# cudagu/aero-gnn

Hardware: AMD Instinct MI355X
Metric: million edge-updates/sec, 1M-node/6M-edge mesh, 1->8 MI355X (higher is better)
Workload: dtype bf16; 1 GPU; BSMS-MGN 4-scale U-Net train step (fwd+MSE+bwd+allreduce+Adam), 1000000 nodes / 5996000 edges per GPU; model=BiStridedMeshGraphNet(H=128, n_hid=2, processor_size=15, stride=2, concat_trick), mode=train, global_batch=1, parallelism=dp1

## Files before the change

### aero-gnn_amd/aerognn/_lib.py

```python
from __future__ import annotations

import ctypes as C
import os

_HERE = os.path.dirname(os.path.abspath(__file__))
LIB_PATH = os.environ.get("AEROGNN_LIB") or os.path.join(_HERE, "libaerognn.so")

MAX_LIN = 8
MAX_SEG = 3
F32, BF16, F16, F64 = 0, 1, 2, 3
SEG_PLAIN, SEG_GATHER, SEG_SUM, SEG_MEAN = 0, 1, 2, 3
OPT_RESIDENT = 0

vp = C.c_void_p
i32 = C.c_int


class Seg(C.Structure):
    _fields_ = [("kind", i32), ("k", i32), ("ld", i32), ("_pad", i32),
                ("ptr", vp), ("index", vp), ("store", vp)]


ACT = {"relu": 0, "gelu": 1, "silu": 2, "tanh": 3}

# ... 17 lines not shown
                ("hpre", vp), ("stats", vp), ("ln_g", vp),
                ("g", vp), ("g2", vp), ("gidx", vp),
                ("gpre", vp * MAX_LIN),
                ("din_nseg", i32), ("din_k", i32 * MAX_SEG),
                ("din", vp * MAX_SEG), ("din_resid", i32 * MAX_SEG),
                ("ln_partial", vp), ("tiled", i32), ("gpre_tiled", i32),
                ("mask", vp * MAX_LIN), ("act_fn", i32), ("_pad3", i32), ("pre", vp * MAX_LIN)]


MAX_WGRAD = 8


class WgradDesc(C.Structure):
    _fields_ = [("g", vp), ("x", vp), ("ldg", i32), ("ldx", i32), ("m", i32), ("k", i32), ("rows", i32),
                ("ldw", i32), ("dw_partial", vp), ("db_partial", vp), ("dw", vp), ("db", vp),
                ("g_tiled", i32), ("x_tiled", i32), ("nsplit", i32), ("_pad", i32), ("xidx", vp)]


class WgradBatch(C.Structure):
    _fields_ = [("n", i32), ("_pad", i32), ("d", WgradDesc * MAX_WGRAD)]


class WecArgs(C.Structure):
    _fields_ = [("n", i32), ("e", i32), ("dtype", i32), ("out_dim", i32), ("hid", i32), ("pos_dim", i32),
                ("pos_ld", i32), ("mean", i32),
                ("rowptr", vp), ("src", vp), ("dst", vp), ("perm", vp), ("rowptr_src", vp), ("perm_src", vp),
                ("pos", vp), ("pab", vp), ("tx", vp), ("w1c", vp), ("w2", vp),
                ("w_in", vp), ("w_out", vp), ("out", vp), ("dout", vp), ("gw", vp), ("s_csc", vp), ("dh", vp),
                ("dpa", vp), ("dpb", vp), ("dtx", vp), ("dw_in", vp), ("partial", vp)]


# ... 199 lines not shown
```

### aero-gnn_amd/aerognn/core.py

```python
from __future__ import annotations

import ctypes as C

import torch

from . import _lib as L
from ._lib import check, ptr


def stream():
    return C.c_void_p(torch.cuda.current_stream().cuda_stream)


PROF = None
_TIMED_DEPTH = 0


class _Timed:
    __slots__ = ("tag", "cost", "s", "on")

    def __init__(self, tag, cost):
        self.tag, self.cost = tag, cost
        self.on = False

# ... 477 lines not shown


def scatter_rows(idx32, src, out):
    check(L.lib().agn_scatter_rows(idx32.numel(), src.shape[1], dt_code(src.dtype), ptr(idx32), ptr(src),
                                   src.stride(0), ptr(out), out.stride(0), stream()), "scatter_rows")
    return out


def colsum_rows(p, nw, n, out):
    sr = min(512, max(1, nw))
    scratch = torch.empty(sr * n, dtype=torch.float32, device=p.device)
    check(L.lib().agn_colsum(ptr(p), nw, n, ptr(scratch), sr, ptr(out), stream()), "colsum")
    return out


class WGrad:

    def __init__(self, tag="wgrad"):
        self.items = []
        self.tag = tag

    def add(self, G, X, dw, db=None, xidx=None):
        assert G.dtype == X.dtype and logical_rows(G) == (logical_rows(X) if xidx is None else xidx.numel())
        assert dw.dtype == torch.float32 and dw.stride(1) == 1
        assert xidx is None or (xidx.dtype == torch.int32 and not is_tiled(X))
        self.items.append((G, X, dw, db, xidx))

    def run(self):
        lib = L.lib()
        plain = [it for it in self.items if it[4] is None]
        gath = [it for it in self.items if it[4] is not None]
        chunks = [grp[i:i + L.MAX_WGRAD] for grp in (plain, gath) for i in range(0, len(grp), L.MAX_WGRAD)]
        for chunk in chunks:
            dev = chunk[0][0].device
            live = []
            for G, X, dw, db, xi in chunk:
                if logical_rows(G) == 0:
                    dw.zero_()
                    if db is not None:
                        db.zero_()
                else:
                    live.append((G, X, dw, db, xi))
            if not live:
                continue
            b = L.WgradBatch()
            b.n = len(live)
            for j, (G, X, dw, db, xi) in enumerate(live):
                b.d[j] = L.WgradDesc(ptr(G), ptr(X), G.stride(0), X.stride(0), G.shape[1], X.shape[1], logical_rows(G),
                                     dw.stride(0), None, None, ptr(dw), ptr(db), int(is_tiled(G)), int(is_tiled(X)), 0, 0,
                                     ptr(xi))
            check(lib.agn_wgrad_plan(C.byref(b)), "wgrad_plan")
            sizes = [int(lib.agn_wgrad_partial_floats(G.shape[1], X.shape[1], b.d[j].nsplit))
                     for j, (G, X, _, _, _) in enumerate(live)]
            bsz = [b.d[j].nsplit * ((G.shape[1] + 127) // 128) * 128 if db is not None else 0
                   for j, (G, _, _, db, _) in enumerate(live)]
            scratch = torch.empty(sum(sizes) + sum(bsz), dtype=torch.float32, device=dev)
            o = 0
            for j, (G, X, dw, db, _) in enumerate(live):
                b.d[j].dw_partial = ptr(scratch[o:o + sizes[j]])
                o += sizes[j]
                if db is not None:
                    b.d[j].db_partial = ptr(scratch[o:o + bsz[j]])
                    o += bsz[j]
            s_el = live[0][0].element_size()
            io = sum(logical_rows(G) * (G.shape[1] + X.shape[1]) * s_el + 4 * G.shape[1] * (X.shape[1] + 1)
                     for G, X, _, _, _ in live)
            fl = sum(2.0 * logical_rows(G) * G.shape[1] * X.shape[1] for G, X, _, _, _ in live)
            with timed(self.tag, (0.0, fl, io)):
                check(lib.agn_wgrad(C.byref(b), dt_code(live[0][0].dtype), 0, stream()), "wgrad")
        self.items = []


def alg8d_edge(E, N, H, s, bwd=False):
    return (2 if bwd else 1) * (E * (2 * s * H + 8) + N * 2 * s * H)


def alg8d_node(N, H, s, bwd=False, proj=False):
    return (2 if bwd else 1) * N * 3 * s * H * (2 if (bwd and proj) else 1)


def with_alg(alg, impl):
    return (alg, impl[1], impl[0])


# ... 57 lines not shown
```

### aero-gnn_amd/aerognn/functions.py

```python
from __future__ import annotations

import ctypes as C

import torch

from . import _lib as L
from ._lib import check, ptr
from . import core as _core
from .core import (Pack, WGrad, alg8d_edge, alg8d_node, with_alg, edge_bwd_fused, fused_edge_train_ok, bwd_nblocks,
                   edge32_ok, edge_saves_ok, edge_forward,
                   cost_edge_bwd_fused,
                   proj_kernel_ok, proj_forward, proj_backward, tiled_empty, relu_mask_empty, colsum_rows, cost_edge_bwd, cost_edge_bwd_cat, cost_edge_fwd,
                   cost_edge_fwd_cat, cost_node_bwd, cost_node_fwd, cost_proj, cost_wec_bwd, cost_wec_fwd, dt_code,
                   timed, gather_rows, mlp_backward, mlp_forward, require_device,
                   scatter_rows, segment_max, segment_max_backward, segment_sum, segment_sum2, stream)


def _c(t):
    return t if t.is_contiguous() else t.contiguous()


def _ln_grads(partial, nblk, M, dtype):
    out = torch.empty(2 * M, dtype=torch.float32, device=partial.device)
    colsum_rows(partial, nblk, 2 * M, out)
# ... 73 lines not shown
        stats = torch.empty(rows, 2, dtype=torch.float32, device=dev)
    return acts, hpre, stats


def _alloc_gpre(spec, rows, dtype, dev, rowmajor=()):
    out = []
    for l in range(spec.nlin):
        w = spec.hidden if l < spec.nlin - 1 else spec.out_dim
        if w == spec.hidden == 128 and l not in rowmajor:
            out.append(tiled_empty(rows, w, dtype, dev))
        else:
            out.append(torch.empty(rows, w, dtype=dtype, device=dev))
    return out


def _chain_param_grads(spec, gpre, inputs0, acts, lnp_partial, nblk, wg=None, tag="wgrad_enc"):
    own = wg is None
    wg = wg or WGrad(tag)
    grads = []
    dev = gpre[0].device
    for l, (w, b) in enumerate(spec.linears):
        G = gpre[l]
        M, K = w.shape
        dw = torch.empty(M, K, dtype=torch.float32, device=dev)
        db = torch.empty(M, dtype=torch.float32, device=dev) if b is not None else None
        if l == 0 and isinstance(inputs0, (list, tuple)):
            k0 = 0
            for j, X in enumerate(inputs0):
                X, xi = X if isinstance(X, tuple) else (X, None)
                wg.add(G, X, dw[:, k0:k0 + X.shape[1]], db if j == 0 else None, xidx=xi)
                k0 += X.shape[1]
        else:
            wg.add(G, inputs0 if l == 0 else acts[l - 1], dw, db)
        grads.append((dw, w.dtype))
        if b is not None:
            grads.append((db, b.dtype))
    if own:
        wg.run()
    out = [g if g.dtype == dt else g.to(dt) for g, dt in grads]
    if spec.ln is not None:
        g, bb = _ln_grads(lnp_partial, nblk, spec.out_dim, spec.ln[0].dtype)
# ... 332 lines not shown
                dxs = torch.empty(E, H, dtype=dt, device=dev)
                dxd = torch.empty(E, H, dtype=dt, device=dev)
                din = [(H, dxs, False), (H, dxd, False), (H, de, True)] if spec.gmp_order else \
                    [(H, de, True), (H, dxs, False), (H, dxd, False)]
            nb_e = mlp_backward(rows=E, dtype=dt, hidden=H, nlin=es.nlin, act_fn=es.act, out_dim=H, in_dim=es.in_dim,
                                wtpk=es.wtpk(), acts=ea, g=ge, g2=dagg, gidx=lv.dst, gpre=gpre_e,
                                ln_g=es.lnp()[0] if es.ln else None, hpre=ehp, stats=est, din=din, ln_partial=part_e,
                                tag="edge_bwd",
                                cost=with_alg(alg8d_edge(E, N, H, sz, bwd=True),
                                              (cost_edge_bwd if spec.trick else cost_edge_bwd_cat)(E, N, H, sz,
                                                                                                   es.nlin)))
            g0 = gpre_e[0]
        grads_edge = []
        if spec.trick:
            dPs = segment_sum(N, H, lv.rowptr_src, lv.perm_src, g0, torch.empty(N, H, dtype=dt, device=dev))
            dPd = segment_sum(N, H, lv.rowptr, None, g0, torch.empty(N, H, dtype=dt, device=dev))
            if proj_kernel_ok(dx, H):
                s_el = dx.element_size()
                proj_backward(N, dPs, dPd, spec.pack["projT"], dx, tag="proj_bwd",
                              cost=with_alg(alg8d_node(N, H, s_el, bwd=True), (4 * N * H * s_el, 4.0 * N * H * H)))
            else:
                mlp_forward(rows=N, dtype=dt, hidden=H, nlin=1, out_dim=H,
                            segs=[(L.SEG_PLAIN, H, H, dPs, None, None), (L.SEG_PLAIN, H, H, dPd, None, None)],
                            wpk=[spec.pack["projT"]], bias=[None], resid=dx, out=dx)
            eb = spec.eb
            wg = WGrad("wgrad_node")
            if fused:
                dwe = torch.empty(H, H, dtype=torch.float32, device=dev)
                we = WGrad("wgrad_edge")
                we.add(g0, e, dwe)
                we.run()
                eg = [dwe]
                for l in range(3):
                    eg += [dW13[l], db13[l]]
                eg = eg[:1] + [t if t.dtype == p.dtype else t.to(p.dtype) for t, p in zip(eg[1:], es.params()[1:7])]
                eg += list(_ln_grads(part_e, nb_e, H, es.ln[0].dtype))
            else:
                eg = _chain_param_grads(es, gpre_e, e, ea, part_e, nb_e, tag="wgrad_edge")
            dws = torch.empty(H, x.shape[1], dtype=torch.float32, device=dev)
            dwd = torch.empty(H, x.shape[1], dtype=torch.float32, device=dev)
            dbd = torch.empty(H, dtype=torch.float32, device=dev)
            wg.add(dPs, x, dws)
            wg.add(dPd, x, dwd, dbd)
            grads_node = _chain_param_grads(ns, gpre_n, [x, agg], na, part_n, nb_n, wg)
            wg.run()
            if fused and eg[0].dtype != es.linears[0][0].dtype:
                eg[0] = eg[0].to(es.linears[0][0].dtype)
            grads_edge = [eg[0], dws.to(eb.src_lin.dtype), dwd.to(eb.dst_lin.dtype), dbd.to(eb.bias.dtype)] + eg[1:]
            return (dx, de, None, None, None, *grads_edge, *grads_node)
        else:
            segment_sum2(N, H, dx, (lv.rowptr_src, lv.perm_src, dxs), (lv.rowptr, None, dxd), dx)
            xs, xd = (x, lv.src), (x, lv.dst)
            grads_edge = _chain_param_grads(es, gpre_e, [xs, xd, e] if spec.gmp_order else [e, xs, xd],
# ... 141 lines not shown
        nb = bwd_nblocks(E)
        part = torch.empty(nb, 2 * H, dtype=torch.float32, device=dev) if es.ln else None
        de = torch.empty_like(e)
        if spec.trick:
            din = [(H, de, False)]
        else:
            dxs = torch.empty(E, H, dtype=dt, device=dev)
            dxd = torch.empty(E, H, dtype=dt, device=dev)
            din = [(H, de, False), (H, dxs, False), (H, dxd, False)]
        nb = mlp_backward(rows=E, dtype=dt, hidden=H, nlin=es.nlin, act_fn=es.act, out_dim=H, in_dim=es.in_dim, wtpk=es.wtpk(),
                     acts=ea, g=g, gpre=gpre, ln_g=es.lnp()[0] if es.ln else None, hpre=ehp, stats=est,
                     din=din, ln_partial=part)
        if spec.trick:
            g0 = gpre[0]
            dPs = segment_sum(N, H, lv.rowptr_src, lv.perm_src, g0, torch.empty(N, H, dtype=dt, device=dev))
            dPd = segment_sum(N, H, lv.rowptr, None, g0, torch.empty(N, H, dtype=dt, device=dev))
            dx = torch.zeros_like(x)
            mlp_forward(rows=N, dtype=dt, hidden=H, nlin=1, out_dim=H,
                        segs=[(L.SEG_PLAIN, H, H, dPs, None, None), (L.SEG_PLAIN, H, H, dPd, None, None)],
                        wpk=[spec.pack["projT"]], bias=[None], out=dx)
            eg = _chain_param_grads(es, gpre, e, ea, part, nb, tag="wgrad_edge")
            eb = spec.eb
            wg = WGrad("wgrad_node")
            dws = torch.empty(H, x.shape[1], dtype=torch.float32, device=dev)
            dwd = torch.empty(H, x.shape[1], dtype=torch.float32, device=dev)
            dbd = torch.empty(H, dtype=torch.float32, device=dev)
            wg.add(dPs, x, dws)
            wg.add(dPd, x, dwd, dbd)
            wg.run()
            grads = [eg[0], dws.to(eb.src_lin.dtype), dwd.to(eb.dst_lin.dtype), dbd.to(eb.bias.dtype)] + eg[1:]
        else:
            dx = segment_sum2(N, H, None, (lv.rowptr_src, lv.perm_src, dxs), (lv.rowptr, None, dxd),
                              torch.empty(N, H, dtype=dt, device=dev))
            grads = _chain_param_grads(es, gpre, [e, (x, lv.src), (x, lv.dst)], ea, part, nb, tag="wgrad_edge")
        return (dx, de, None, None, None, *grads)

# ... 321 lines not shown
```

### aero-gnn_amd/csrc/dw.hip

```cpp
#include "common.hpp"
#include "aerognn.h"

#include <type_traits>

using namespace agn;

namespace {

#ifndef AGN_DW_ROWS
#define AGN_DW_ROWS 64
#endif
constexpr int DW_ROWS = AGN_DW_ROWS;
constexpr int DW_BLK = 128;
constexpr int DW_THREADS = 256;

typedef short s16x4 __attribute__((ext_vector_type(4)));
typedef __attribute__((address_space(3))) s16x4 lds_s16x4;

template <typename T> struct DwTile;
template <> struct DwTile<bf16> { static constexpr int LD = 136; };
template <> struct DwTile<f16> { static constexpr int LD = 136; };
template <> struct DwTile<float> { static constexpr int LD = 132; };

template <typename T>
// ... 57 lines not shown
#pragma unroll
            for (int e = 0; e < 4; ++e)
              if (4 + e < nv) e4[e] = p[4 + e];
            const u32x2 hi = *reinterpret_cast<const u32x2*>(e4);
            v[j] = __builtin_bit_cast(uint4, u32x4{lo[0], lo[1], hi[0], hi[1]});
          } else {
            T e8[PER16];
#pragma unroll
            for (int e = 0; e < PER16; ++e) e8[e] = e < nv ? p[e] : from_f<T>(0.f);
            v[j] = *reinterpret_cast<const uint4*>(e8);
          }
        }
      }
    }
  }
  AGN_DEV void store(T* lds, int tiled) const {
    constexpr int LD = DwTile<T>::LD;
    if (tiled) {
#pragma unroll
      for (int j = 0; j < NCH; ++j) {
        int row, i, hh;
        tiled_pos(threadIdx.x + j * DW_THREADS, row, i, hh);
        if constexpr (sizeof(T) == 2) {
          const u32x4 x = __builtin_bit_cast(u32x4, v[j]);
          typedef uint32_t u32x2 __attribute__((ext_vector_type(2)));
          *reinterpret_cast<u32x2*>(lds + row * LD + 16 * i + 4 * hh) = u32x2{x[0], x[1]};
          *reinterpret_cast<u32x2*>(lds + row * LD + 16 * i + 8 + 4 * hh) = u32x2{x[2], x[3]};
        } else {
          *reinterpret_cast<uint4*>(lds + row * LD + 8 * i + 4 * hh) = v[j];
        }
// ... 12 lines not shown
AGN_DEV bf16x8 tr_frag(const bf16* lds, int kb, int col_base, int lane) {
  constexpr int LD = DwTile<bf16>::LD;
  const int q = (lane & 15) >> 2, p = lane & 3;
  const bf16* a0 = lds + (kb + q) * LD + col_base + 4 * p;
  const bf16* a1 = a0 + 4 * LD;
  s16x4 lo = __builtin_amdgcn_ds_read_tr16_b64_v4i16((lds_s16x4*)(a0));
  s16x4 hi = __builtin_amdgcn_ds_read_tr16_b64_v4i16((lds_s16x4*)(a1));
  bf16x8 r;
  const bf16x4 l4 = *reinterpret_cast<const bf16x4*>(&lo);
  const bf16x4 h4 = *reinterpret_cast<const bf16x4*>(&hi);
  r[0] = l4[0]; r[1] = l4[1]; r[2] = l4[2]; r[3] = l4[3];
  r[4] = h4[0]; r[5] = h4[1]; r[6] = h4[2]; r[7] = h4[3];
  return r;
}

template <typename T, bool XG>
__global__ __launch_bounds__(DW_THREADS) void wgrad_kernel(const agn_wgrad_batch b, int nsplit) {
  constexpr int LD = DwTile<T>::LD;
  __shared__ __attribute__((aligned(16))) T sg[DW_ROWS * LD];
  __shared__ __attribute__((aligned(16))) T sx[DW_ROWS * LD];
  const agn_wgrad_desc& d = b.d[blockIdx.z];
  const int nKb = (d.k + DW_BLK - 1) / DW_BLK;
  const int nMb = (d.m + DW_BLK - 1) / DW_BLK;
  if ((int)blockIdx.y >= nMb * nKb) return;
  const int mb = blockIdx.y / nKb, kb = blockIdx.y % nKb;
  const int m0 = mb * DW_BLK, k0 = kb * DW_BLK;
  const int split = blockIdx.x;
  const int per = ((d.rows + nsplit - 1) / nsplit + DW_ROWS - 1) / DW_ROWS * DW_ROWS;
  const int rbeg = split * per, rend = min(d.rows, rbeg + per);
  const int lane = threadIdx.x & 63, w = threadIdx.x >> 6;
  const int wm = (w >> 1) * 64, wk = (w & 1) * 64;
  const T* G = reinterpret_cast<const T*>(d.g);
  const T* X = reinterpret_cast<const T*>(d.x);
  f32x16 acc[2][2];
#pragma unroll
  for (int i = 0; i < 2; ++i)
#pragma unroll
    for (int j = 0; j < 2; ++j) acc[i][j] = f32x16{};
  float bsum = 0.f;
  __shared__ float bhalf[DW_BLK];
  StageRegs<T> rg, rx;
  if (rbeg < rend) {
    rg.load(G, d.ldg, rend, d.m, rbeg, m0, d.g_tiled);
    rx.load(X, d.ldx, rend, d.k, rbeg, k0, d.x_tiled, XG ? d.xidx : nullptr);
  }
  for (int r0 = rbeg; r0 < rend; r0 += DW_ROWS) {
    __syncthreads();
    rg.store(sg, d.g_tiled);
    rx.store(sx, d.x_tiled);
    __syncthreads();
    if (r0 + DW_ROWS < rend) {
      rg.load(G, d.ldg, rend, d.m, r0 + DW_ROWS, m0, d.g_tiled);
      rx.load(X, d.ldx, rend, d.k, r0 + DW_ROWS, k0, d.x_tiled, XG ? d.xidx : nullptr);
    }
    if (d.db_partial && kb == 0) {
      const int col = threadIdx.x & (DW_BLK - 1), q = threadIdx.x >> 7;
#pragma unroll
      for (int gq = 0; gq < DW_ROWS / 32; ++gq)
#pragma unroll 8
        for (int r = 0; r < 16; ++r) bsum += to_f(sg[(32 * gq + 16 * q + r) * LD + col]);
    }
    if constexpr (sizeof(T) == 2) {
#pragma unroll
      for (int ks = 0; ks < DW_ROWS; ks += 16) {
        const int kbase = ks + 8 * (lane >> 5);
        bf16x8 a[2], bb[2];
#pragma unroll
        for (int i = 0; i < 2; ++i) a[i] = tr_frag(reinterpret_cast<const bf16*>(sg), kbase, wm + 32 * i + 16 * ((lane >> 4) & 1), lane);
#pragma unroll
        for (int j = 0; j < 2; ++j) bb[j] = tr_frag(reinterpret_cast<const bf16*>(sx), kbase, wk + 32 * j + 16 * ((lane >> 4) & 1), lane);
#pragma unroll
        for (int i = 0; i < 2; ++i)
#pragma unroll
          for (int j = 0; j < 2; ++j) {
            if constexpr (std::is_same<T, f16>::value)
              acc[i][j] = __builtin_amdgcn_mfma_f32_32x32x16_f16(__builtin_bit_cast(f16x8, a[i]),
                                                                 __builtin_bit_cast(f16x8, bb[j]), acc[i][j], 0, 0, 0);
            else
              acc[i][j] = __builtin_amdgcn_mfma_f32_32x32x16_bf16(a[i], bb[j], acc[i][j], 0, 0, 0);
          }
      }
    } else {
      const float* fg = reinterpret_cast<const float*>(sg);
      const float* fx = reinterpret_cast<const float*>(sx);
#pragma unroll 4
      for (int ks = 0; ks < DW_ROWS; ks += 2) {
        const int r = ks + (lane >> 5), cidx = lane & 31;
        float a[2], bb[2];
#pragma unroll
        for (int i = 0; i < 2; ++i) a[i] = fg[r * LD + wm + 32 * i + cidx];
#pragma unroll
        for (int j = 0; j < 2; ++j) bb[j] = fx[r * LD + wk + 32 * j + cidx];
#pragma unroll
        for (int i = 0; i < 2; ++i)
#pragma unroll
          for (int j = 0; j < 2; ++j) acc[i][j] = __builtin_amdgcn_mfma_f32_32x32x2f32(a[i], bb[j], acc[i][j], 0, 0, 0);
      }
    }
  }
  const int kpad = nKb * DW_BLK;
  float* P = d.dw_partial + (size_t)split * (nMb * DW_BLK) * kpad;
#pragma unroll
  for (int i = 0; i < 2; ++i)
#pragma unroll
    for (int j = 0; j < 2; ++j)
#pragma unroll
      for (int r = 0; r < 16; ++r) {
        const int m = m0 + wm + 32 * i + (r & 3) + 8 * (r >> 2) + 4 * (lane >> 5);
        const int k = k0 + wk + 32 * j + (lane & 31);
        P[(size_t)m * kpad + k] = acc[i][j][r];
      }
  if (d.db_partial && kb == 0) {
    __syncthreads();
    if (threadIdx.x >= DW_BLK) bhalf[threadIdx.x - DW_BLK] = bsum;
    __syncthreads();
    if (threadIdx.x < DW_BLK) d.db_partial[(size_t)split * (nMb * DW_BLK) + m0 + threadIdx.x] = bsum + bhalf[threadIdx.x];
  }
}

constexpr int RED_G = 8;
constexpr int RED_Q = 16;
__global__ __launch_bounds__(RED_Q * RED_G) void wgrad_reduce_kernel(const agn_wgrad_batch b) {
  __shared__ f32x4 part[RED_G][RED_Q];
  __shared__ float bpart[RED_G][RED_Q];
  const agn_wgrad_desc& d = b.d[blockIdx.y];
  const int nsplit = d.nsplit;
  const int nKb = (d.k + DW_BLK - 1) / DW_BLK, nMb = (d.m + DW_BLK - 1) / DW_BLK;
  const int kpad = nKb * DW_BLK, mpad = nMb * DW_BLK;
  const size_t slab = (size_t)mpad * kpad;
  const int kq = kpad / 4;
  const int t = threadIdx.x % RED_Q, g = threadIdx.x / RED_Q;
  const int qidx = blockIdx.x * RED_Q + t;
  const bool in_slab = qidx < mpad * kq;
  f32x4 s = {0.f, 0.f, 0.f, 0.f};
  if (in_slab) {
    const float* p = d.dw_partial + (size_t)qidx * 4;
    int sp = g;
    for (; sp + 3 * RED_G < nsplit; sp += 4 * RED_G) {
      f32x4 v[4];
#pragma unroll
      for (int j = 0; j < 4; ++j) v[j] = *reinterpret_cast<const f32x4*>(p + (size_t)(sp + j * RED_G) * slab);
// ... 83 lines not shown
  hipError_t e = hipGetLastError();
  return e == hipSuccess ? 0 : (int)e;
}

}

extern "C" {

namespace {
int wgrad_resident() {
  static int resident = 0;
  if (resident == 0) {
    int dev = 0, ncu = 256, per = 3;
    hipDeviceProp_t p;
    if (hipGetDevice(&dev) == hipSuccess && hipGetDeviceProperties(&p, dev) == hipSuccess) ncu = p.multiProcessorCount;
    if (hipOccupancyMaxActiveBlocksPerMultiprocessor(&per, wgrad_kernel<bf16, false>, DW_THREADS, 0) != hipSuccess || per < 1)
      per = 3;
    resident = ncu * per;
  }
  return resident;
}
int out_blocks(const agn_wgrad_desc& d) { return ((d.m + DW_BLK - 1) / DW_BLK) * ((d.k + DW_BLK - 1) / DW_BLK); }
}

int agn_wgrad_nsplit(int rows, int ndesc_blocks) {
  int ns = wgrad_resident() / (ndesc_blocks > 0 ? ndesc_blocks : 1);
  const int maxs = (rows + 2 * DW_ROWS - 1) / (2 * DW_ROWS);
  if (ns > maxs) ns = maxs;
  return ns < 1 ? 1 : ns;
}

// ... 6 lines not shown
  if (!b || b->n < 1 || b->n > AGN_MAX_WGRAD) return AGN_E_ARG;
  int nblk = 0, rows = 0;
  for (int i = 0; i < b->n; ++i) {
    nblk += out_blocks(b->d[i]);
    rows = b->d[i].rows > rows ? b->d[i].rows : rows;
  }
  const int ns = agn_wgrad_nsplit(rows, nblk);
  for (int i = 0; i < b->n; ++i) b->d[i].nsplit = ns;
  return 0;
}

int agn_wgrad(const agn_wgrad_batch* b, int dtype, int nsplit, void* stream) {
  if (!b || b->n < 1 || b->n > AGN_MAX_WGRAD) return AGN_E_ARG;
  agn_wgrad_batch bb = *b;
  int total = 0, maxq = 1;
  for (int i = 0; i < bb.n; ++i) {
    agn_wgrad_desc& d = bb.d[i];
    if (d.m < 1 || d.k < 1 || d.rows < 0) return AGN_E_ARG;
    if ((d.g_tiled && d.m != DW_BLK) || (d.x_tiled && d.k != DW_BLK)) return AGN_E_SHAPE;
    if (d.xidx && d.x_tiled) return AGN_E_ARG;
    if (nsplit > 0) d.nsplit = nsplit;
    if (d.nsplit < 1) return AGN_E_ARG;
    total += out_blocks(d) * d.nsplit;
    const int kpad = ((d.k + DW_BLK - 1) / DW_BLK) * DW_BLK, mpad = ((d.m + DW_BLK - 1) / DW_BLK) * DW_BLK;
    maxq = mpad * kpad / 4 > maxq ? mpad * kpad / 4 : maxq;
  }
  hipStream_t st = (hipStream_t)stream;
  const int ns = bb.d[0].nsplit;
  int maxblk = 1;
  for (int i = 0; i < bb.n; ++i) {
    if (bb.d[i].nsplit != ns) return AGN_E_ARG;
    maxblk = out_blocks(bb.d[i]) > maxblk ? out_blocks(bb.d[i]) : maxblk;
  }
  (void)total;
  dim3 grid(ns, maxblk, bb.n);
  bool xg = false;
  for (int i = 0; i < bb.n; ++i) xg = xg || bb.d[i].xidx != nullptr;
#define AGN_WG(T)                                                                             \
  do {                                                                                        \
    if (xg) hipLaunchKernelGGL((wgrad_kernel<T, true>), grid, dim3(DW_THREADS), 0, st, bb, ns); \
    else hipLaunchKernelGGL((wgrad_kernel<T, false>), grid, dim3(DW_THREADS), 0, st, bb, ns);   \
  } while (0)
  if (dtype == AGN_BF16) AGN_WG(bf16);
  else if (dtype == AGN_F16) AGN_WG(f16);
  else if (dtype == AGN_F32) AGN_WG(float);
  else return AGN_E_DTYPE;
#undef AGN_WG
  hipLaunchKernelGGL(wgrad_reduce_kernel, dim3((maxq + RED_Q - 1) / RED_Q, bb.n), dim3(RED_Q * RED_G), 0, st, bb);
  return launch_status();
}

int agn_wgrad_reduce(const agn_wgrad_batch* b, int nsplit, void* stream) {
  if (!b || b->n < 1 || b->n > AGN_MAX_WGRAD || nsplit < 1) return AGN_E_ARG;
  agn_wgrad_batch bb = *b;
  int maxq = 1;
  for (int i = 0; i < bb.n; ++i) {
    bb.d[i].nsplit = nsplit;
    const int kpad = ((bb.d[i].k + DW_BLK - 1) / DW_BLK) * DW_BLK;
    const int mpad = ((bb.d[i].m + DW_BLK - 1) / DW_BLK) * DW_BLK;
    maxq = mpad * kpad / 4 > maxq ? mpad * kpad / 4 : maxq;
  }
  hipLaunchKernelGGL(wgrad_reduce_kernel, dim3((maxq + RED_Q - 1) / RED_Q, bb.n), dim3(RED_Q * RED_G), 0, (hipStream_t)stream, bb);
  return launch_status();
}

int agn_colsum(const float* p, int nw, int n, float* scratch, int scratch_rows, float* out, void* stream) {
  if (nw < 0 || n < 1 || scratch_rows < 1) return AGN_E_ARG;
  hipStream_t st = (hipStream_t)stream;
  if (nw == 0) {
    hipError_t e = hipMemsetAsync(out, 0, sizeof(float) * n, st);
    return e == hipSuccess ? 0 : (int)e;
  }
  const int chunk = (nw + scratch_rows - 1) / scratch_rows;
  const int nc = (nw + chunk - 1) / chunk;
  hipLaunchKernelGGL(colsum_stage1, dim3((n + 255) / 256, nc), dim3(256), 0, st, p, nw, n, chunk, scratch);
  hipLaunchKernelGGL(colsum_stage2, dim3((n + 63) / 64), dim3(64 * RED_G), 0, st, scratch, nc, n, out);
  return launch_status();
// ... 4 lines not shown
```

### include/aerognn.h

```cpp
#ifndef AEROGNN_H
#define AEROGNN_H
#include <stddef.h>
#include <stdint.h>
#ifdef __cplusplus
extern "C" {
#endif

#define AGN_MAX_LIN 8
#define AGN_MAX_SEG 3

enum { AGN_F32 = 0, AGN_BF16 = 1, AGN_F16 = 2, AGN_F64 = 3 };
enum { AGN_SEG_PLAIN = 0, AGN_SEG_GATHER = 1, AGN_SEG_SUM = 2, AGN_SEG_MEAN = 3 };
enum { AGN_E_ARG = -1, AGN_E_DTYPE = -2, AGN_E_HIDDEN = -3, AGN_E_SHAPE = -4 };
enum { AGN_ACT_RELU = 0, AGN_ACT_GELU = 1, AGN_ACT_SILU = 2, AGN_ACT_TANH = 3 };

typedef struct {
  int kind;
  int k;
  int ld;
  int _pad;
  const void* ptr;
  const int32_t* index;
  void* store;
} agn_seg;
// ... 77 lines not shown
#define AGN_MAX_WGRAD 8
typedef struct {
  const void* g;
  const void* x;
  int ldg, ldx;
  int m, k, rows;
  int ldw;
  float* dw_partial;
  float* db_partial;
  float* dw;
  float* db;
  int g_tiled, x_tiled;
  int nsplit;
  int _pad;
  const int32_t* xidx;
} agn_wgrad_desc;
typedef struct {
  int n;
  int _pad;
  agn_wgrad_desc d[AGN_MAX_WGRAD];
} agn_wgrad_batch;
int agn_wgrad_nsplit(int rows, int ndesc_blocks);
size_t agn_wgrad_partial_floats(int m, int k, int nsplit);
int agn_wgrad_plan(agn_wgrad_batch* b);
int agn_wgrad(const agn_wgrad_batch* b, int dtype, int nsplit, void* stream);
int agn_colsum(const float* p, int nw, int n, float* scratch, int scratch_rows, float* out, void* stream);

int agn_version(void);
const char* agn_error_string(int code);
enum {
// ... 218 lines not shown
```

Baseline: 777.1 M edge-updates/s.

## Fuse receiver segment-sum of edge gradients into edge weight-gradient kernel

Computes the destination-node segment sum of the first edge-MLP gradient (dPd) inside the wgrad kernel. It reuses the G tiles already staged in LDS and uses MFMA with a one-hot segment matrix, so a separate segment_sum pass over the edge gradients is no longer needed. Segments that span split boundaries are carried through scratch and combined in the reduce kernel. The cost is a more complex kernel with extra LDS, a changed occupancy hint, and boundary-handling logic that could hurt wgrad throughput or correctness.

```diff
diff --git a/aero-gnn_amd/aerognn/_lib.py b/aero-gnn_amd/aerognn/_lib.py
--- a/aero-gnn_amd/aerognn/_lib.py
+++ b/aero-gnn_amd/aerognn/_lib.py
@@ -55,7 +55,8 @@
 class WgradDesc(C.Structure):
     _fields_ = [("g", vp), ("x", vp), ("ldg", i32), ("ldx", i32), ("m", i32), ("k", i32), ("rows", i32),
                 ("ldw", i32), ("dw_partial", vp), ("db_partial", vp), ("dw", vp), ("db", vp),
-                ("g_tiled", i32), ("x_tiled", i32), ("nsplit", i32), ("_pad", i32), ("xidx", vp)]
+                ("g_tiled", i32), ("x_tiled", i32), ("nsplit", i32), ("_pad", i32), ("xidx", vp),
+                ("seg_dst", vp), ("seg_out", vp), ("seg_scratch", vp), ("seg_n", i32), ("_pad2", i32)]
 
 
 class WgradBatch(C.Structure):
diff --git a/aero-gnn_amd/aerognn/core.py b/aero-gnn_amd/aerognn/core.py
--- a/aero-gnn_amd/aerognn/core.py
+++ b/aero-gnn_amd/aerognn/core.py
@@ -515,60 +515,86 @@
     return out
 
 
+def wgrad_seg_ok(G, X) -> bool:
+    return (G.dtype in (torch.bfloat16, torch.float16) and not is_tiled(G) and not is_tiled(X)
+            and G.shape[1] == 128 and X.shape[1] == 128 and G.stride(0) % 8 == 0 and X.stride(0) % 8 == 0
+            and G.stride(1) == 1 and X.stride(1) == 1 and G.data_ptr() % 16 == 0 and X.data_ptr() % 16 == 0)
+
+
 class WGrad:
 
-    def __init__(self, tag="wgrad"):
+    def __init__(self, tag="wgrad", nsplit=0):
         self.items = []
+        self.nsplit = int(nsplit)
         self.tag = tag
 
-    def add(self, G, X, dw, db=None, xidx=None):
+    def add(self, G, X, dw, db=None, xidx=None, seg=None):
         assert G.dtype == X.dtype and logical_rows(G) == (logical_rows(X) if xidx is None else xidx.numel())
         assert dw.dtype == torch.float32 and dw.stride(1) == 1
         assert xidx is None or (xidx.dtype == torch.int32 and not is_tiled(X))
-        self.items.append((G, X, dw, db, xidx))
+        if seg is not None:
+            dst, out = seg
+            if not wgrad_seg_ok(G, X) or xidx is not None:
+                raise ValueError("aerognn: receiver sums need row-major 16-bit G and X of width 128")
+            assert dst.dtype == torch.int32 and dst.numel() == G.shape[0]
+            assert out.dtype == G.dtype and out.shape[1] == 128 and out.is_contiguous()
+        self.items.append((G, X, dw, db, xidx, seg))
 
     def run(self):
         lib = L.lib()
-        plain = [it for it in self.items if it[4] is None]
+        plain = [it for it in self.items if it[4] is None and it[5] is None]
         gath = [it for it in self.items if it[4] is not None]
         chunks = [grp[i:i + L.MAX_WGRAD] for grp in (plain, gath) for i in range(0, len(grp), L.MAX_WGRAD)]
+        chunks += [[it] for it in self.items if it[5] is not None]
         for chunk in chunks:
             dev = chunk[0][0].device
             live = []
-            for G, X, dw, db, xi in chunk:
+            for G, X, dw, db, xi, seg in chunk:
                 if logical_rows(G) == 0:
                     dw.zero_()
                     if db is not None:
                         db.zero_()
+                    if seg is not None:
+                        seg[1].zero_()
                 else:
-                    live.append((G, X, dw, db, xi))
+                    live.append((G, X, dw, db, xi, seg))
             if not live:
                 continue
             b = L.WgradBatch()
             b.n = len(live)
-            for j, (G, X, dw, db, xi) in enumerate(live):
+            for j, (G, X, dw, db, xi, seg) in enumerate(live):
                 b.d[j] = L.WgradDesc(ptr(G), ptr(X), G.stride(0), X.stride(0), G.shape[1], X.shape[1], logical_rows(G),
                                      dw.stride(0), None, None, ptr(dw), ptr(db), int(is_tiled(G)), int(is_tiled(X)), 0, 0,
                                      ptr(xi))
             check(lib.agn_wgrad_plan(C.byref(b)), "wgrad_plan")
-            sizes = [int(lib.agn_wgrad_partial_floats(G.shape[1], X.shape[1], b.d[j].nsplit))
-                     for j, (G, X, _, _, _) in enumerate(live)]
-            bsz = [b.d[j].nsplit * ((G.shape[1] + 127) // 128) * 128 if db is not None else 0
-                   for j, (G, _, _, db, _) in enumerate(live)]
-            scratch = torch.empty(sum(sizes) + sum(bsz), dtype=torch.float32, device=dev)
+            if self.nsplit > 0:
+                for j in range(b.n):
+                    b.d[j].nsplit = self.nsplit
+            sizes = [int(lib.agn_wgrad_partial_floats(it[0].shape[1], it[1].shape[1], b.d[j].nsplit))
+                     for j, it in enumerate(live)]
+            bsz = [b.d[j].nsplit * ((it[0].shape[1] + 127) // 128) * 128 if it[3] is not None else 0
+                   for j, it in enumerate(live)]
+            ssz = [256 * b.d[j].nsplit if it[5] is not None else 0 for j, it in enumerate(live)]
+            scratch = torch.empty(sum(sizes) + sum(bsz) + sum(ssz), dtype=torch.float32, device=dev)
             o = 0
-            for j, (G, X, dw, db, _) in enumerate(live):
+            for j, (G, X, dw, db, _, seg) in enumerate(live):
                 b.d[j].dw_partial = ptr(scratch[o:o + sizes[j]])
                 o += sizes[j]
                 if db is not None:
                     b.d[j].db_partial = ptr(scratch[o:o + bsz[j]])
                     o += bsz[j]
+                if seg is not None:
+                    b.d[j].seg_dst, b.d[j].seg_out = ptr(seg[0]), ptr(seg[1])
+                    b.d[j].seg_n = seg[1].shape[0]
+                    b.d[j].seg_scratch = ptr(scratch[o:o + ssz[j]])
+                    o += ssz[j]
             s_el = live[0][0].element_size()
             io = sum(logical_rows(G) * (G.shape[1] + X.shape[1]) * s_el + 4 * G.shape[1] * (X.shape[1] + 1)
-                     for G, X, _, _, _ in live)
-            fl = sum(2.0 * logical_rows(G) * G.shape[1] * X.shape[1] for G, X, _, _, _ in live)
+                     + (4 * logical_rows(G) + seg[1].numel() * s_el if seg is not None else 0)
+                     for G, X, _, _, _, seg in live)
+            fl = sum(2.0 * logical_rows(G) * G.shape[1] * X.shape[1] for G, X, _, _, _, _ in live)
             with timed(self.tag, (0.0, fl, io)):
-                check(lib.agn_wgrad(C.byref(b), dt_code(live[0][0].dtype), 0, stream()), "wgrad")
+                check(lib.agn_wgrad(C.byref(b), dt_code(live[0][0].dtype), self.nsplit, stream()), "wgrad")
         self.items = []
 
 
diff --git a/aero-gnn_amd/aerognn/functions.py b/aero-gnn_amd/aerognn/functions.py
--- a/aero-gnn_amd/aerognn/functions.py
+++ b/aero-gnn_amd/aerognn/functions.py
@@ -7,7 +7,7 @@
 from . import _lib as L
 from ._lib import check, ptr
 from . import core as _core
-from .core import (Pack, WGrad, alg8d_edge, alg8d_node, with_alg, edge_bwd_fused, fused_edge_train_ok, bwd_nblocks,
+from .core import (Pack, WGrad, wgrad_seg_ok, alg8d_edge, alg8d_node, with_alg, edge_bwd_fused, fused_edge_train_ok, bwd_nblocks,
                    edge32_ok, edge_saves_ok, edge_forward,
                    cost_edge_bwd_fused,
                    proj_kernel_ok, proj_forward, proj_backward, tiled_empty, relu_mask_empty, colsum_rows, cost_edge_bwd, cost_edge_bwd_cat, cost_edge_fwd,
@@ -111,7 +111,20 @@
     return out
 
 
-def _chain_param_grads(spec, gpre, inputs0, acts, lnp_partial, nblk, wg=None, tag="wgrad_enc"):
+def edge_dw_dpd(g0, e, lv, N, dw, db=None):
+    H = g0.shape[1]
+    dPd = torch.empty(N, H, dtype=g0.dtype, device=g0.device)
+    we = WGrad("wgrad_edge")
+    if wgrad_seg_ok(g0, e):
+        we.add(g0, e, dw, db, seg=(lv.dst, dPd))
+    else:
+        segment_sum(N, H, lv.rowptr, None, g0, dPd)
+        we.add(g0, e, dw, db)
+    we.run()
+    return dPd
+
+
+def _chain_param_grads(spec, gpre, inputs0, acts, lnp_partial, nblk, wg=None, tag="wgrad_enc", first=None):
     own = wg is None
     wg = wg or WGrad(tag)
     grads = []
@@ -121,7 +134,9 @@
         M, K = w.shape
         dw = torch.empty(M, K, dtype=torch.float32, device=dev)
         db = torch.empty(M, dtype=torch.float32, device=dev) if b is not None else None
-        if l == 0 and isinstance(inputs0, (list, tuple)):
+        if l == 0 and first is not None:
+            dw, db = first
+        elif l == 0 and isinstance(inputs0, (list, tuple)):
             k0 = 0
             for j, X in enumerate(inputs0):
                 X, xi = X if isinstance(X, tuple) else (X, None)
@@ -484,7 +499,9 @@
         grads_edge = []
         if spec.trick:
             dPs = segment_sum(N, H, lv.rowptr_src, lv.perm_src, g0, torch.empty(N, H, dtype=dt, device=dev))
-            dPd = segment_sum(N, H, lv.rowptr, None, g0, torch.empty(N, H, dtype=dt, device=dev))
+            dwe = torch.empty(H, H, dtype=torch.float32, device=dev)
+            dbe = torch.empty(H, dtype=torch.float32, device=dev) if es.linears[0][1] is not None else None
+            dPd = edge_dw_dpd(g0, e, lv, N, dwe, dbe)
             if proj_kernel_ok(dx, H):
                 s_el = dx.element_size()
                 proj_backward(N, dPs, dPd, spec.pack["projT"], dx, tag="proj_bwd",
@@ -496,17 +513,13 @@
             eb = spec.eb
             wg = WGrad("wgrad_node")
             if fused:
-                dwe = torch.empty(H, H, dtype=torch.float32, device=dev)
-                we = WGrad("wgrad_edge")
-                we.add(g0, e, dwe)
-                we.run()
                 eg = [dwe]
                 for l in range(3):
                     eg += [dW13[l], db13[l]]
                 eg = eg[:1] + [t if t.dtype == p.dtype else t.to(p.dtype) for t, p in zip(eg[1:], es.params()[1:7])]
                 eg += list(_ln_grads(part_e, nb_e, H, es.ln[0].dtype))
             else:
-                eg = _chain_param_grads(es, gpre_e, e, ea, part_e, nb_e, tag="wgrad_edge")
+                eg = _chain_param_grads(es, gpre_e, e, ea, part_e, nb_e, tag="wgrad_edge", first=(dwe, dbe))
             dws = torch.empty(H, x.shape[1], dtype=torch.float32, device=dev)
             dwd = torch.empty(H, x.shape[1], dtype=torch.float32, device=dev)
             dbd = torch.empty(H, dtype=torch.float32, device=dev)
@@ -678,12 +691,14 @@
         if spec.trick:
             g0 = gpre[0]
             dPs = segment_sum(N, H, lv.rowptr_src, lv.perm_src, g0, torch.empty(N, H, dtype=dt, device=dev))
-            dPd = segment_sum(N, H, lv.rowptr, None, g0, torch.empty(N, H, dtype=dt, device=dev))
+            dwe = torch.empty(H, H, dtype=torch.float32, device=dev)
+            dbe = torch.empty(H, dtype=torch.float32, device=dev) if es.linears[0][1] is not None else None
+            dPd = edge_dw_dpd(g0, e, lv, N, dwe, dbe)
             dx = torch.zeros_like(x)
             mlp_forward(rows=N, dtype=dt, hidden=H, nlin=1, out_dim=H,
                         segs=[(L.SEG_PLAIN, H, H, dPs, None, None), (L.SEG_PLAIN, H, H, dPd, None, None)],
                         wpk=[spec.pack["projT"]], bias=[None], out=dx)
-            eg = _chain_param_grads(es, gpre, e, ea, part, nb, tag="wgrad_edge")
+            eg = _chain_param_grads(es, gpre, e, ea, part, nb, tag="wgrad_edge", first=(dwe, dbe))
             eb = spec.eb
             wg = WGrad("wgrad_node")
             dws = torch.empty(H, x.shape[1], dtype=torch.float32, device=dev)
diff --git a/aero-gnn_amd/csrc/dw.hip b/aero-gnn_amd/csrc/dw.hip
--- a/aero-gnn_amd/csrc/dw.hip
+++ b/aero-gnn_amd/csrc/dw.hip
@@ -95,6 +95,25 @@
       }
     }
   }
+  AGN_DEV void load_rows(const T* __restrict__ g, int ld, int rows, int r0, int tid) {
+#pragma unroll
+    for (int j = 0; j < NCH; ++j) {
+      const int i = tid + j * DW_THREADS;
+      const int r = i / CHUNKS, ch = i - r * CHUNKS;
+      const T* base = g + (size_t)r0 * ld;
+      const uint32_t off = (uint32_t)(r * ld + ch * PER16);
+      v[j] = (r0 + r < rows) ? *reinterpret_cast<const uint4*>(base + off) : uint4{0u, 0u, 0u, 0u};
+    }
+  }
+  AGN_DEV void store_rows(T* lds, int tid) const {
+    constexpr int LD = DwTile<T>::LD;
+#pragma unroll
+    for (int j = 0; j < NCH; ++j) {
+      const int i = tid + j * DW_THREADS;
+      const int r = i / CHUNKS, ch = i - r * CHUNKS;
+      *reinterpret_cast<uint4*>(lds + r * LD + ch * PER16) = v[j];
+    }
+  }
   AGN_DEV void store(T* lds, int tiled) const {
     constexpr int LD = DwTile<T>::LD;
     if (tiled) {
@@ -137,11 +156,33 @@
   return r;
 }
 
-template <typename T, bool XG>
-__global__ __launch_bounds__(DW_THREADS) void wgrad_kernel(const agn_wgrad_batch b, int nsplit) {
+template <bool SEG> struct SegSh {};
+template <> struct SegSh<true> {
+  __attribute__((aligned(16))) short sl[DW_ROWS][4];
+  __attribute__((aligned(16))) int sid[DW_ROWS];
+  int meta[2];
+  float carry[2][DW_BLK];
+  float head[DW_BLK];
+};
+template <typename T> struct SegOne;
+template <> struct SegOne<bf16> { static constexpr uint32_t v = 0x3f80u; };
+template <> struct SegOne<f16> { static constexpr uint32_t v = 0x3c00u; };
+template <> struct SegOne<float> { static constexpr uint32_t v = 0u; };
+template <typename P> AGN_DEV P* uni_ptr(P* p) {
+  const uint64_t v = reinterpret_cast<uint64_t>(p);
+  const uint32_t lo = __builtin_amdgcn_readfirstlane((uint32_t)v), hi = __builtin_amdgcn_readfirstlane((uint32_t)(v >> 32));
+  return reinterpret_cast<P*>(((uint64_t)hi << 32) | lo);
+}
+AGN_DEV uint32_t seg_sel(uint32_t two, uint32_t tgt, uint32_t one) {
+  return ((two & 0xffffu) == tgt ? one : 0u) | ((two >> 16) == tgt ? one << 16 : 0u);
+}
+
+template <typename T, bool XG, bool SEG>
+__global__ __launch_bounds__(DW_THREADS, SEG ? 3 : 1) void wgrad_kernel(const agn_wgrad_batch b, int nsplit) {
   constexpr int LD = DwTile<T>::LD;
   __shared__ __attribute__((aligned(16))) T sg[DW_ROWS * LD];
   __shared__ __attribute__((aligned(16))) T sx[DW_ROWS * LD];
+  __shared__ SegSh<SEG> ss;
   const agn_wgrad_desc& d = b.d[blockIdx.z];
   const int nKb = (d.k + DW_BLK - 1) / DW_BLK;
   const int nMb = (d.m + DW_BLK - 1) / DW_BLK;
@@ -163,18 +204,155 @@
   float bsum = 0.f;
   __shared__ float bhalf[DW_BLK];
   StageRegs<T> rg, rx;
+  [[maybe_unused]] bool seg = false, head_wg = false, tail_wg = false, cont_in = false;
+  [[maybe_unused]] int s_dc = 0, s_dn = 0, id0 = -1;
+  [[maybe_unused]] const int32_t* sdst = nullptr;
+  [[maybe_unused]] T* sout = nullptr;
+  [[maybe_unused]] const int sb = __builtin_amdgcn_readfirstlane(w & 1);
+  if constexpr (SEG) {
+    seg = d.seg_out != nullptr && rbeg < rend;
+    if (seg) {
+      sdst = uni_ptr(d.seg_dst);
+      sout = uni_ptr(reinterpret_cast<T*>(d.seg_out));
+      id0 = sdst[rbeg];
+      head_wg = rbeg > 0 && sdst[rbeg - 1] == id0;
+      tail_wg = rend < d.rows && sdst[rend] == sdst[rend - 1];
+      if (w == 0) {
+        s_dc = sdst[(uint32_t)min(rbeg + lane, d.rows - 1)];
+        s_dn = sdst[(uint32_t)min(rbeg + lane + 1, d.rows - 1)];
+        if (rbeg == 0)
+          for (int row = lane >> 4; row < id0; row += 4)
+            *reinterpret_cast<uint4*>(sout + (size_t)row * DW_BLK + (lane & 15) * 8) = uint4{0u, 0u, 0u, 0u};
+      }
+    }
+  }
   if (rbeg < rend) {
-    rg.load(G, d.ldg, rend, d.m, rbeg, m0, d.g_tiled);
-    rx.load(X, d.ldx, rend, d.k, rbeg, k0, d.x_tiled, XG ? d.xidx : nullptr);
+    if constexpr (SEG) {
+      rg.load_rows(G, d.ldg, rend, rbeg, threadIdx.x);
+      rx.load_rows(X, d.ldx, rend, rbeg, threadIdx.x);
+    } else {
+      rg.load(G, d.ldg, rend, d.m, rbeg, m0, d.g_tiled);
+      rx.load(X, d.ldx, rend, d.k, rbeg, k0, d.x_tiled, XG ? d.xidx : nullptr);
+    }
   }
   for (int r0 = rbeg; r0 < rend; r0 += DW_ROWS) {
     __syncthreads();
-    rg.store(sg, d.g_tiled);
-    rx.store(sx, d.x_tiled);
+    [[maybe_unused]] int tl = threadIdx.x, ln = lane;
+    if constexpr (SEG) {
+      asm volatile("" : "+v"(tl));
+      rg.store_rows(sg, tl);
+      rx.store_rows(sx, tl);
+    } else {
+      rg.store(sg, d.g_tiled);
+      rx.store(sx, d.x_tiled);
+    }
+    [[maybe_unused]] unsigned long long gapmask = 0;
+    [[maybe_unused]] int gap_lo = 0, gap_hi = 0;
+    if constexpr (SEG) {
+      if (seg && w == 0) {
+        const int r = r0 + lane;
+        const bool valid = r < rend;
+        const bool bnd = valid && lane < DW_ROWS - 1 && r + 1 < rend && s_dn != s_dc;
+        const unsigned long long bm = __ballot(bnd);
+        const int slot = __popcll(bm & ((1ull << lane) - 1ull));
+        const short s16 = (short)slot;
+        *reinterpret_cast<s16x4*>(&ss.sl[lane][0]) = s16x4{s16, s16, s16, s16};
+        if (valid && (lane == 0 || ((bm >> (lane - 1)) & 1ull))) ss.sid[slot] = s_dc;
+        if (lane == DW_ROWS - 1) {
+          ss.meta[0] = __popcll(bm) + 1;
+          ss.meta[1] = (r0 + DW_ROWS < rend && s_dn == s_dc) ? 1 : 0;
+        }
+        gap_lo = s_dc + 1;
+        gap_hi = (r + 1 < d.rows) ? s_dn : d.seg_n;
+        gapmask = __ballot(valid && gap_hi > gap_lo);
+      }
+    }
     __syncthreads();
     if (r0 + DW_ROWS < rend) {
-      rg.load(G, d.ldg, rend, d.m, r0 + DW_ROWS, m0, d.g_tiled);
-      rx.load(X, d.ldx, rend, d.k, r0 + DW_ROWS, k0, d.x_tiled, XG ? d.xidx : nullptr);
+      if constexpr (SEG) {
+        if (seg && w == 0) {
+          s_dc = sdst[(uint32_t)min(r0 + DW_ROWS + lane, d.rows - 1)];
+          s_dn = sdst[(uint32_t)min(r0 + DW_ROWS + lane + 1, d.rows - 1)];
+        }
+        rg.load_rows(G, d.ldg, rend, r0 + DW_ROWS, tl);
+        rx.load_rows(X, d.ldx, rend, r0 + DW_ROWS, tl);
+      } else {
+        rg.load(G, d.ldg, rend, d.m, r0 + DW_ROWS, m0, d.g_tiled);
+        rx.load(X, d.ldx, rend, d.k, r0 + DW_ROWS, k0, d.x_tiled, XG ? d.xidx : nullptr);
+      }
+    }
+    if constexpr (SEG) {
+      while (gapmask) {
+        const int src = __ffsll((long long)gapmask) - 1;
+        gapmask &= gapmask - 1ull;
+        const int lo = __shfl(gap_lo, src), hi = __shfl(gap_hi, src);
+        for (int row = lo + (lane >> 4); row < hi; row += 4)
+          *reinterpret_cast<uint4*>(sout + (size_t)row * DW_BLK + (lane & 15) * 8) = uint4{0u, 0u, 0u, 0u};
+      }
+    }
+    [[maybe_unused]] f32x16 pacc = f32x16{};
+    [[maybe_unused]] auto seg_frag = [&](auto& sh, int kbase) {
+      const int q = (ln & 15) >> 2;
+      const s16x4 lo = __builtin_amdgcn_ds_read_tr16_b64_v4i16((lds_s16x4*)(&sh.sl[kbase + q][0]));
+      const s16x4 hi = __builtin_amdgcn_ds_read_tr16_b64_v4i16((lds_s16x4*)(&sh.sl[kbase + q + 4][0]));
+      typedef uint32_t u32x2 __attribute__((ext_vector_type(2)));
+      const u32x2 l2 = __builtin_bit_cast(u32x2, lo), h2 = __builtin_bit_cast(u32x2, hi);
+      const uint32_t tgt = 32 * sb + (ln & 31);
+      constexpr uint32_t one = SegOne<T>::v;
+      return u32x4{seg_sel(l2[0], tgt, one), seg_sel(l2[1], tgt, one), seg_sel(h2[0], tgt, one), seg_sel(h2[1], tgt, one)};
+    };
+    [[maybe_unused]] auto seg_mfma = [&](const u32x4& sv, const bf16x8& g) {
+      if constexpr (std::is_same<T, f16>::value)
+        pacc = __builtin_amdgcn_mfma_f32_32x32x16_f16(__builtin_bit_cast(f16x8, sv), __builtin_bit_cast(f16x8, g), pacc, 0, 0, 0);
+      else
+        pacc = __builtin_amdgcn_mfma_f32_32x32x16_bf16(__builtin_bit_cast(bf16x8, sv), g, pacc, 0, 0, 0);
+    };
+    [[maybe_unused]] auto seg_flush = [&](auto& sh, int i, int ns, bool keep_last, bool head0) {
+      const int par = ((r0 - rbeg) / DW_ROWS) & 1;
+      const int col = wm + 32 * i + (ln & 31);
+      if (cont_in && sb == 0 && ln < 32) pacc[0] = sh.carry[par][col] + pacc[0];
+#pragma unroll
+      for (int j = 0; j < 4; ++j) {
+        const int mj = 32 * sb + 8 * j;
+        if (mj < ns) {
+          const int m0s = mj + 4 * (ln >> 5);
+          typedef int i32x4 __attribute__((ext_vector_type(4)));
+          const i32x4 ids = *reinterpret_cast<const i32x4*>(&sh.sid[m0s]);
+#pragma unroll
+          for (int q = 0; q < 4; ++q) {
+            const int m = m0s + q;
+            if (m < ns) {
+              const float v = pacc[4 * j + q];
+              if (m == ns - 1 && keep_last) sh.carry[par ^ 1][col] = v;
+              else if (m == 0 && head0) sh.head[col] = v;
+              else
+                *reinterpret_cast<T*>(reinterpret_cast<char*>(sout) + (uint32_t)(ids[q] * (DW_BLK * 2) + col * 2)) = from_f<T>(v);
+            }
+          }
+        }
+        __builtin_amdgcn_sched_barrier(0);
+      }
+    };
+    if constexpr (SEG) {
+      if (seg) {
+        const int ns = __builtin_amdgcn_readfirstlane(ss.meta[0]);
+        const bool cont_out = __builtin_amdgcn_readfirstlane(ss.meta[1]) != 0;
+        const bool keep_last = cont_out || (tail_wg && r0 + DW_ROWS >= rend);
+        asm volatile("" : "+v"(ln));
+        const bool head0 = head_wg && __builtin_amdgcn_readfirstlane(ss.sid[0]) == id0;
+#pragma unroll 1
+        for (int i = 0; i < 2 && 32 * sb < ns; ++i) {
+          pacc = f32x16{};
+#pragma unroll
+          for (int ks = 0; ks < DW_ROWS; ks += 16) {
+            const int kbase = ks + 8 * (ln >> 5);
+            seg_mfma(seg_frag(ss, kbase), tr_frag(reinterpret_cast<const bf16*>(sg), kbase, wm + 32 * i + 16 * ((ln >> 4) & 1), ln));
+          }
+          seg_flush(ss, i, ns, keep_last, head0);
+        }
+        cont_in = cont_out;
+        __builtin_amdgcn_sched_barrier(0);
+      }
     }
     if (d.db_partial && kb == 0) {
       const int col = threadIdx.x & (DW_BLK - 1), q = threadIdx.x >> 7;
@@ -202,6 +380,7 @@
             else
               acc[i][j] = __builtin_amdgcn_mfma_f32_32x32x16_bf16(a[i], bb[j], acc[i][j], 0, 0, 0);
           }
+        if constexpr (SEG) __builtin_amdgcn_sched_barrier(0);
       }
     } else {
       const float* fg = reinterpret_cast<const float*>(sg);
@@ -221,6 +400,17 @@
       }
     }
   }
+  if constexpr (SEG) {
+    if (seg && (head_wg || tail_wg)) {
+      __syncthreads();
+      if (threadIdx.x < DW_BLK) {
+        float* Hs = d.seg_scratch + (size_t)split * (2 * DW_BLK);
+        const int par = (((rend - rbeg - 1) / DW_ROWS) & 1) ^ 1;
+        if (tail_wg) Hs[(head_wg && sdst[rend - 1] == id0 ? 0 : DW_BLK) + threadIdx.x] = ss.carry[par][threadIdx.x];
+        if (head_wg && !(tail_wg && sdst[rend - 1] == id0)) Hs[threadIdx.x] = ss.head[threadIdx.x];
+      }
+    }
+  }
   const int kpad = nKb * DW_BLK;
   float* P = d.dw_partial + (size_t)split * (nMb * DW_BLK) * kpad;
 #pragma unroll
@@ -243,11 +433,33 @@
 
 constexpr int RED_G = 8;
 constexpr int RED_Q = 16;
-__global__ __launch_bounds__(RED_Q * RED_G) void wgrad_reduce_kernel(const agn_wgrad_batch b) {
+__global__ __launch_bounds__(RED_Q * RED_G) void wgrad_reduce_kernel(const agn_wgrad_batch b, int seg_dt) {
+  static_assert(RED_Q * RED_G == DW_BLK, "one thread per receiver-sum column");
   __shared__ f32x4 part[RED_G][RED_Q];
   __shared__ float bpart[RED_G][RED_Q];
   const agn_wgrad_desc& d = b.d[blockIdx.y];
   const int nsplit = d.nsplit;
+  if (seg_dt >= 0 && d.seg_out && d.rows > 0) {
+    const int per = ((d.rows + nsplit - 1) / nsplit + DW_ROWS - 1) / DW_ROWS * DW_ROWS;
+    const int32_t* sd = d.seg_dst;
+    for (int s = blockIdx.x; s < nsplit; s += gridDim.x) {
+      const long long rbeg = (long long)s * per;
+      const long long rend = rbeg + per;
+      if (rend >= d.rows) break;
+      const int v = sd[rend - 1];
+      if (sd[rend] != v) continue;
+      if (rbeg > 0 && sd[rbeg - 1] == v) continue;
+      float sum = d.seg_scratch[(size_t)s * (2 * DW_BLK) + DW_BLK + threadIdx.x];
+      for (int j = s + 1; j < nsplit; ++j) {
+        const long long rb = (long long)j * per;
+        if (rb >= d.rows || sd[rb] != v) break;
+        sum += d.seg_scratch[(size_t)j * (2 * DW_BLK) + threadIdx.x];
+      }
+      const size_t o = (size_t)v * DW_BLK + threadIdx.x;
+      if (seg_dt == AGN_BF16) reinterpret_cast<bf16*>(d.seg_out)[o] = from_f<bf16>(sum);
+      else reinterpret_cast<f16*>(d.seg_out)[o] = from_f<f16>(sum);
+    }
+  }
   const int nKb = (d.k + DW_BLK - 1) / DW_BLK, nMb = (d.m + DW_BLK - 1) / DW_BLK;
   const int kpad = nKb * DW_BLK, mpad = nMb * DW_BLK;
   const size_t slab = (size_t)mpad * kpad;
@@ -361,7 +573,7 @@
     int dev = 0, ncu = 256, per = 3;
     hipDeviceProp_t p;
     if (hipGetDevice(&dev) == hipSuccess && hipGetDeviceProperties(&p, dev) == hipSuccess) ncu = p.multiProcessorCount;
-    if (hipOccupancyMaxActiveBlocksPerMultiprocessor(&per, wgrad_kernel<bf16, false>, DW_THREADS, 0) != hipSuccess || per < 1)
+    if (hipOccupancyMaxActiveBlocksPerMultiprocessor(&per, wgrad_kernel<bf16, false, false>, DW_THREADS, 0) != hipSuccess || per < 1)
       per = 3;
     resident = ncu * per;
   }
@@ -398,6 +610,7 @@
   if (!b || b->n < 1 || b->n > AGN_MAX_WGRAD) return AGN_E_ARG;
   agn_wgrad_batch bb = *b;
   int total = 0, maxq = 1;
+  bool seg = false;
   for (int i = 0; i < bb.n; ++i) {
     agn_wgrad_desc& d = bb.d[i];
     if (d.m < 1 || d.k < 1 || d.rows < 0) return AGN_E_ARG;
@@ -405,6 +618,15 @@
     if (d.xidx && d.x_tiled) return AGN_E_ARG;
     if (nsplit > 0) d.nsplit = nsplit;
     if (d.nsplit < 1) return AGN_E_ARG;
+    if (d.seg_out || d.seg_dst || d.seg_scratch) {
+      if (!d.seg_out || !d.seg_dst || !d.seg_scratch || d.seg_n < 0 || (d.rows > 0 && d.seg_n < 1)) return AGN_E_ARG;
+      if (dtype != AGN_BF16 && dtype != AGN_F16) return AGN_E_DTYPE;
+      if (d.g_tiled || d.x_tiled || d.xidx) return AGN_E_ARG;
+      if (d.m != DW_BLK || d.k != DW_BLK) return AGN_E_SHAPE;
+      if (d.seg_n > (1 << 23)) return AGN_E_SHAPE;
+      if ((d.ldg % 8) || (d.ldx % 8) || ((uintptr_t)d.g & 15) || ((uintptr_t)d.x & 15)) return AGN_E_ARG;
+      seg = true;
+    }
     total += out_blocks(d) * d.nsplit;
     const int kpad = ((d.k + DW_BLK - 1) / DW_BLK) * DW_BLK, mpad = ((d.m + DW_BLK - 1) / DW_BLK) * DW_BLK;
     maxq = mpad * kpad / 4 > maxq ? mpad * kpad / 4 : maxq;
@@ -420,17 +642,30 @@
   dim3 grid(ns, maxblk, bb.n);
   bool xg = false;
   for (int i = 0; i < bb.n; ++i) xg = xg || bb.d[i].xidx != nullptr;
+  if (seg && xg) return AGN_E_ARG;
+  if (seg) {
+    for (int i = 0; i < bb.n; ++i) {
+      const agn_wgrad_desc& d = bb.d[i];
+      if (d.seg_out && d.rows == 0 && d.seg_n > 0 &&
+          hipMemsetAsync(d.seg_out, 0, (size_t)d.seg_n * DW_BLK * 2, st) != hipSuccess)
+        return launch_status();
+    }
+    if (dtype == AGN_BF16) hipLaunchKernelGGL((wgrad_kernel<bf16, false, true>), grid, dim3(DW_THREADS), 0, st, bb, ns);
+    else hipLaunchKernelGGL((wgrad_kernel<f16, false, true>), grid, dim3(DW_THREADS), 0, st, bb, ns);
+    hipLaunchKernelGGL(wgrad_reduce_kernel, dim3((maxq + RED_Q - 1) / RED_Q, bb.n), dim3(RED_Q * RED_G), 0, st, bb, dtype);
+    return launch_status();
+  }
 #define AGN_WG(T)                                                                             \
   do {                                                                                        \
-    if (xg) hipLaunchKernelGGL((wgrad_kernel<T, true>), grid, dim3(DW_THREADS), 0, st, bb, ns); \
-    else hipLaunchKernelGGL((wgrad_kernel<T, false>), grid, dim3(DW_THREADS), 0, st, bb, ns);   \
+    if (xg) hipLaunchKernelGGL((wgrad_kernel<T, true, false>), grid, dim3(DW_THREADS), 0, st, bb, ns); \
+    else hipLaunchKernelGGL((wgrad_kernel<T, false, false>), grid, dim3(DW_THREADS), 0, st, bb, ns);   \
   } while (0)
   if (dtype == AGN_BF16) AGN_WG(bf16);
   else if (dtype == AGN_F16) AGN_WG(f16);
   else if (dtype == AGN_F32) AGN_WG(float);
   else return AGN_E_DTYPE;
 #undef AGN_WG
-  hipLaunchKernelGGL(wgrad_reduce_kernel, dim3((maxq + RED_Q - 1) / RED_Q, bb.n), dim3(RED_Q * RED_G), 0, st, bb);
+  hipLaunchKernelGGL(wgrad_reduce_kernel, dim3((maxq + RED_Q - 1) / RED_Q, bb.n), dim3(RED_Q * RED_G), 0, st, bb, -1);
   return launch_status();
 }
 
@@ -444,7 +679,7 @@
     const int mpad = ((bb.d[i].m + DW_BLK - 1) / DW_BLK) * DW_BLK;
     maxq = mpad * kpad / 4 > maxq ? mpad * kpad / 4 : maxq;
   }
-  hipLaunchKernelGGL(wgrad_reduce_kernel, dim3((maxq + RED_Q - 1) / RED_Q, bb.n), dim3(RED_Q * RED_G), 0, (hipStream_t)stream, bb);
+  hipLaunchKernelGGL(wgrad_reduce_kernel, dim3((maxq + RED_Q - 1) / RED_Q, bb.n), dim3(RED_Q * RED_G), 0, (hipStream_t)stream, bb, -1);
   return launch_status();
 }
 
diff --git a/include/aerognn.h b/include/aerognn.h
--- a/include/aerognn.h
+++ b/include/aerognn.h
@@ -115,6 +115,11 @@
   int nsplit;
   int _pad;
   const int32_t* xidx;
+  const int32_t* seg_dst;
+  void* seg_out;
+  float* seg_scratch;
+  int seg_n;
+  int _pad2;
 } agn_wgrad_desc;
 typedef struct {
   int n;
```

Measured after the change: 787.2 M edge-updates/s, median of 6. 1.3% higher.
